# mapillary/OpenSfM

Hardware: NVIDIA H100
Metric: BA observations/sec (higher is better)
Workload: dtype f64

## Files before the change

### opensfm_b200/csrc/ba.cu

```cuda
#include <algorithm>
#include <dlfcn.h>

#include <chrono>
#include <cstring>
#include <mutex>
#include <cmath>
#include <cstdlib>
#include <string>
#include <vector>

#include "ba_models.cuh"
#include "common.cuh"

struct OsfmNcclId { char internal[128]; };

namespace osfm {

struct BAView {
  int K, NI, NR, S, P;
  long long N;
  int nc, npf;
  int wc, nres;
  int loss;
  double loss_a;
// ... 802 lines not shown
  osfm_allreduce_fn allreduce = nullptr;
  void* allreduce_user = nullptr;
  void* nccl_comm = nullptr;
  int nccl_rank = -1, nccl_world = 0;
  bool reproj_valid = false;
  osfm_ba_summary summary{};
  bool has_run = false;
  unsigned fallbacks = 0;
  int cap_iter = 0;
  bool cap_valid = false;
  osfm_ba_capture cap_info{};
  std::vector<double> cap_sbuf, cap_y, cap_scale, cap_diag, cap_grad;
  std::vector<double> cap_cam, cap_inst, cap_rc, cap_pts, cap_ext;
  std::vector<double> cap_side_r, cap_side_J;
  std::vector<int4> cap_upper;
  std::vector<int> cap_blk_off, cap_blk_sz, cap_pt_poff, cap_global_of;
  int cap_nc_pad = 0;
  bool cov_on = false, cov_ran = false, cov_valid = false;
  int cov_status = OSFM_COV_OK;
  double cov_pass_ms = 0.0, cov_chol_ms = 0.0;
  std::vector<double> cov_out;
  DevBuf<double> d_cov;
  DevBuf<int> d_cov_perm, d_cov_inst, d_cov_flags;

  DevBuf<int> d_cam_type, d_cam_off, d_cam_np, d_cam_poff, d_inst_poff, d_rc_poff, d_pt_poff;
  DevBuf<int> d_shot_inst, d_shot_cam, d_shot_rc, d_shot_use_rc, d_obs_shot, d_obs_point;
  DevBuf<double> d_obs_x, d_obs_y, d_obs_isig;
  DevBuf<long long> d_obs_orig, d_pt_start;
  DevBuf<double> d_cam[2], d_inst[2], d_rc[2], d_pts[2];
  DevBuf<double> d_r, d_Jc, d_Jp, d_Sbuf, d_Vinv, d_gp, d_slots;
  DevBuf<double> d_scale, d_colnorm2, d_grad, d_diag, d_y, d_bs_t;
  DevBuf<double> d_px, d_pr, d_pz, d_pp, d_pAp, d_Minv, d_reproj, d_full_pts;
  DevBuf<double> d_Wdef;
  DevBuf<int> d_blk_off, d_blk_sz, d_cam_blk, d_inst_blk, d_rc_blk;
  DevBuf<unsigned long long> d_tkeys, d_skeys, d_skeys2, d_rkeys, d_rkeys2;
  DevBuf<int> d_tvals, d_area, d_offs, d_row_ptr, d_row_col, d_row_off, d_diag_off, d_prior_diag_off;
  DevBuf<int> d_pr_blk, d_pr_local, d_g_obs_shot, d_g_obs_point;
  DevBuf<long long> d_g_pt_start;
  DevBuf<int4> d_upper;
  DevBuf<unsigned> d_count;
  DevBuf<char> d_cub;
  DevBuf<PcgState> d_pcg;
  DevBuf<int> d_seg_start;
  DevBuf<int> d_raw_shot, d_raw_point, d_ptc_full;
  DevBuf<double> d_raw_xy, d_raw_sigma, d_pts_in;
  DevBuf<unsigned long long> d_okeys, d_okeys2, d_pkey, d_pkey2;
  DevBuf<int> d_ovals, d_ovals2, d_pval, d_order, d_inv_order, d_global_of, d_free_flag, d_free_scan, d_head, d_run_head, d_nsel;
  DevBuf<long long> d_kk;
  DevBuf<char> d_seg_flags;
  DevBuf<OrderCounts> d_oc;
  PinnedBuf<OrderCounts> h_oc;
  DevBuf<double> d_rowsJ, d_rowsW, d_rowsY, d_Vig;
  DevBuf<int> d_row_M, d_qoff, d_blk_row, d_cbase, d_colidx, d_row_of, d_grp_b1, d_grp_b2;
  DevBuf<long long> d_rowbase;
  DevBuf<double> d_Spcg, d_Ap;
  PinnedBuf<PcgState> h_pcg;
  DevBuf<int> d_pcg_rowlo;
  DevBuf<int> d_pcg_grplo;
  DevBuf<char> d_grp_shared;
  DevBuf<unsigned long long> d_prof;
  DevBuf<long long> d_tab_off, d_tab_sizes;
  DevBuf<int> d_sp_nch, d_sp_chunk0;
  DevBuf<SchurChunk> d_sp_chunks;
  DevBuf<int> d_sp_ftab;
  DevBuf<int> d_tab;
  DevBuf<double> d_ptsum;
// ... 421 lines not shown
  upload(d_pr_cam_scale, rs.pr_cam_scale, stream); upload(d_pr_pos_inst, rs.pr_pos_inst, stream);
  upload(d_pr_pos_axis, rs.pr_pos_axis, stream); upload(d_pr_pos_col, rs.pr_pos_col, stream);
  upload(d_pr_pos_kind, rs.pr_pos_kind, stream);
  std::vector<double> ev = ext_values, el = ext_lower;
  if (ev.empty()) { ev.assign(1, 0.0); el.assign(1, 0.0); }
  upload(d_ext[0], ev, stream); upload(d_ext[1], ev, stream); upload(d_ext_lower, el, stream);
  upload(d_ext_off, rs.ext_off, stream); upload(d_ext_np, ext_size, stream); upload(d_ext_poff, rs.ext_poff, stream);
  upload(d_ext_blk, rs.ext_blk, stream);
  upload(d_side_terms, side_terms, stream); upload(d_side_consts, side_consts, stream);
  upload(d_side_jofs, rs.side_jofs, stream); upload(d_side_rofs, rs.side_rofs, stream);
  d_side_J.reserve((size_t)rs.side_jofs[NT] + 1); d_side_r.reserve((size_t)rs.side_rofs[NT] + 1);
  std::vector<double> ppd, ppx;
  if (rs.have_pp) {
    ppd.assign(3 * (size_t)Pfull, 0.0); ppx.assign(3 * (size_t)Pfull, 0.0);
    for (size_t q = 0; q < pp_point.size(); ++q) {
      const size_t g = (size_t)pp_point[q];
      for (int j = 0; j < (pp_alt[q] ? 3 : 2); ++j) {
        ppd[3 * g + j] = 1.0 / std::max(pp_sigma[3 * q + j], DBL_EPSILON);
        ppx[3 * g + j] = pp_prior[3 * q + j];
      }
    }
    upload(d_pp_d, ppd, stream); upload(d_pp_x0, ppx, stream);
  }
  OSFM_CUDA(cudaStreamSynchronize(stream));
  upload(d_pr_pos_prior, rs.pr_pos_prior, stream); upload(d_pr_pos_scale, rs.pr_pos_scale, stream);
  const size_t Nz = (size_t)std::max<long long>(rs.N, 1);
  d_r.reserve(nres * Nz); d_Jc.reserve((size_t)nres * wc * Nz); d_Jp.reserve((size_t)nres * 3 * Nz);
  d_Vinv.reserve(6 * (size_t)std::max(npf, 1)); d_gp.reserve(3 * (size_t)std::max(npf, 1));
  d_Vig.reserve(3 * (size_t)std::max(npf, 1)); d_bs_t.reserve(3 * (size_t)std::max(npf, 1));
  const size_t nz = rs.nz;
  d_scale.reserve(nz); d_colnorm2.reserve(nz); d_grad.reserve(nz); d_diag.reserve(nz); d_diag_r.reserve(nz); d_y.reserve(nz);
  d_px.reserve(std::max(nc, 1)); d_pr.reserve(std::max(nc, 1)); d_pz.reserve(std::max(nc, 1));
  d_pp.reserve(std::max(nc, 1)); d_pAp.reserve(std::max(nc, 1));
  d_pcg.reserve(1);
  d_Minv.reserve((size_t)std::max(rs.ngroups, 1) * MAXB * MAXB);
  d_Ap.reserve(std::max(nc, 1));
  d_sc.reserve(1);

  BAView& v = rs.v;
  v.K = rs.K; v.NI = rs.NI; v.NR = rs.NR; v.S = rs.S; v.P = P; v.N = rs.N; v.nc = nc; v.npf = npf; v.wc = wc; v.nres = nres;
  v.loss = loss; v.loss_a = loss_a;
  v.cam_type = d_cam_type.p; v.cam_off = d_cam_off.p; v.cam_np = d_cam_np.p; v.cam_poff = d_cam_poff.p;
  v.inst_poff = d_inst_poff.p; v.rc_poff = d_rc_poff.p; v.pt_poff = d_pt_poff.p;
  v.shot_inst = d_shot_inst.p; v.shot_cam = d_shot_cam.p; v.shot_rc = d_shot_rc.p; v.shot_use_rc = d_shot_use_rc.p;
  v.obs_shot = d_obs_shot.p; v.obs_point = d_obs_point.p; v.obs_x = d_obs_x.p; v.obs_y = d_obs_y.p;
  v.obs_isig = d_obs_isig.p; v.obs_orig = d_obs_orig.p; v.pt_start = d_pt_start.p;
  v.r = d_r.p; v.Jc = d_Jc.p; v.Jp = d_Jp.p;
  PriorView& pv = rs.pv;
  pv.n_cam_rows = rs.add_priors ? (int)rs.pr_cam_param.size() : 0;
  pv.n_pos_rows = rs.add_priors ? (int)rs.pr_pos_inst.size() : 0;
  pv.cam_row_param = d_pr_cam_param.p; pv.cam_row_col = d_pr_cam_col.p; pv.cam_row_log = d_pr_cam_log.p;
  pv.cam_row_prior = d_pr_cam_prior.p; pv.cam_row_scale = d_pr_cam_scale.p;
  pv.pos_row_kind = d_pr_pos_kind.p;
  pv.pos_row_inst = d_pr_pos_inst.p; pv.pos_row_axis = d_pr_pos_axis.p; pv.pos_row_col = d_pr_pos_col.p;
  pv.pos_row_prior = d_pr_pos_prior.p; pv.pos_row_scale = d_pr_pos_scale.p;
  SideView& sv = rs.sv;
  sv.n = NT; sv.terms = d_side_terms.p; sv.consts = d_side_consts.p; sv.jofs = d_side_jofs.p; sv.rofs = d_side_rofs.p;
  sv.J = d_side_J.p; sv.r = d_side_r.p;
  sv.ext_off = d_ext_off.p; sv.ext_np = d_ext_np.p; sv.ext_poff = d_ext_poff.p; sv.ext_blk = d_ext_blk.p;
  rs.ppv = PointPriorView{rs.have_pp ? d_pp_d.p : nullptr, d_pp_x0.p, d_global_of.p};
  rs.bm = BlkMaps{d_cam_blk.p, d_inst_blk.p, d_rc_blk.p};
}

void BA::discover_structure() {
  const int nblk = rs.nblk, nc = rs.nc, NT = rs.NT;
  if (nblk > 0) {
// ... 455 lines not shown
    if (timed) lm_phase(LM_PH_SCHUR, -1);
  }
  if (nc > 0) {
    if (world > 1) allreduce_dev(d_Sbuf.p, (long long)rs.nc_pad + rs.s_upper_total);
    PriorView pall = rs.pv;
    pall.n_cam_rows = (int)rs.pr_cam_param.size();
    pall.n_pos_rows = (int)rs.pr_pos_inst.size();
    const int nall = pall.n_cam_rows + pall.n_pos_rows;
    if (nall > 0) {
      ba_prior_system<<<grid_for(nall, 128), 128, 0, stream>>>(pall, params_of(0), d_scale.p, d_prior_diag_off.p,
                                                              d_S_p, d_rhs_p);
      OSFM_LAUNCH_CHECK();
    }
    if (rs.NT > 0) {
      side_system<<<rs.NT, SIDE_THREADS, 0, stream>>>(rs.sv, rs.v, rs.bm, params_of(0), rs.bsr, d_scale.p, d_S_p, d_rhs_p);
      OSFM_LAUNCH_CHECK();
    }
    ba_finish_system<<<grid_for((long long)rs.n_upper * 32, 256), 256, 0, stream>>>(d_upper.p, rs.n_upper, rs.bsr, d_S_p,
                                                                                  diag, inv_radius);
    OSFM_LAUNCH_CHECK();
  }
}

void BA::solve_reduced() {
  const int nc = rs.nc;
  lm_phase(-1, LM_PH_PCG);
  pcg_convert<<<grid_for((long long)rs.n_blocks_all * 32, 256), 256, 0, stream>>>(
      rs.d_S_p, d_row_col.p, d_row_off.p, d_qoff.p, d_blk_row.p, rs.n_blocks_all, rs.bsr, d_row_M.p, d_rowbase.p, d_Spcg.p);
  OSFM_LAUNCH_CHECK();
  pcg_factor_groups<<<grid_for((long long)rs.ngroups * 32, 32 * PFG_WARPS), 32 * PFG_WARPS, 0, stream>>>(rs.d_S_p, rs.bsr, d_diag_off.p, d_grp_b1.p, d_grp_b2.p,
                                                                rs.ngroups, d_Minv.p);
  OSFM_LAUNCH_CHECK();
  OSFM_CUDA(cudaMemsetAsync(d_pcg.p, 0, sizeof(PcgState), stream));
  const int max_pcg = std::min(2 * nc + 100, 5000);
  const int classic_path = rs.pcg_resident ? OSFM_PCG_CLASSIC_RESIDENT : OSFM_PCG_CLASSIC_STREAMED;
  auto classic = [&]() {
    launch_cooperative(rs.pcg_resident ? pcg_persistent<true> : pcg_persistent<false>, rs.pcg_grid, PCG_THREADS, rs.pcg_smem,
                       stream, d_Spcg.p, rs.lay, rs.bsr, d_Minv.p, rs.d_rhs_p, d_px.p, d_pr.p, d_pz.p, d_pp.p, d_pAp.p, d_Ap.p,
                       d_pcg.p, nc, max_pcg, 1e-16, rs.pcg_res);
    OSFM_LAUNCH_CHECK();
    if (tracing()) {
      OSFM_CUDA(cudaMemcpyAsync(h_pcg.p, d_pcg.p, PCG_STATE_HEADER, cudaMemcpyDeviceToHost, stream));
      OSFM_CUDA(cudaStreamSynchronize(stream));
      const PcgState& h = *h_pcg.p;
      const int its = std::max(h.iterations, 1);
      fprintf(stderr, "[osfm_ba] pcg %d its, CTA0 clocks/it: stage %lld matvec %lld reduce1 %lld phaseB %lld reduce2 %lld (resident %d)\n",
              h.iterations, h.prof[0] / its, h.prof[1] / its, h.prof[2] / its, h.prof[3] / its, h.prof[4] / its, (int)rs.pcg_resident);
    }
  };
  if (rs.pcg_pipe_ok) {
    launch_cooperative(pcg_pipelined, rs.pcg_grid, PCG_THREADS, rs.pcg_pipe_smem, stream, d_Spcg.p, rs.lay, rs.bsr, d_Minv.p,
                       rs.d_rhs_p, d_px.p, d_pz.p, d_pp.p, d_pcg.p, nc, max_pcg, 1e-16, rs.pcg_pipe);
    OSFM_LAUNCH_CHECK();
    if (tracing()) {
      OSFM_CUDA(cudaMemcpyAsync(h_pcg.p, d_pcg.p, PCG_STATE_HEADER, cudaMemcpyDeviceToHost, stream));
      OSFM_CUDA(cudaStreamSynchronize(stream));
      const PcgState& h = *h_pcg.p;
      const int its = std::max(h.iterations, 1);
      fprintf(stderr, "[osfm_ba] pipelined pcg %d its converged %d, CTA0 clocks/it: stage %lld matvec %lld reduce %lld update %lld"
              " | wide barrier (all calls / its): own sums %lld release %lld collect %lld column sums %lld\n",
              h.iterations, h.converged, h.prof[0] / its, h.prof[1] / its, h.prof[2] / its, h.prof[3] / its, h.prof[4] / its,
              h.prof[5] / its, h.prof[6] / its, h.prof[7] / its);
    }
    ba_lm_pcg_check<<<1, 1, 0, stream>>>(d_lm.p, d_pcg.p, classic_path, rs.h_pcg, rs.cap_graph != nullptr);
    OSFM_LAUNCH_CHECK();
    rs.k_pcg = lm_if(rs.h_pcg, LM_PCG_CLASSIC, [&]() {
      OSFM_CUDA(cudaMemsetAsync(d_pcg.p, 0, sizeof(PcgState), stream));
      classic();
    });
  } else {
    classic();
  }
  OSFM_CUDA(cudaMemcpyAsync(d_y.p, d_px.p, sizeof(double) * nc, cudaMemcpyDeviceToDevice, stream));
  lm_phase(LM_PH_PCG, -1);
}

void BA::back_substitute() {
  const int P = rs.P, npf = rs.npf;
  if (P == 0 || npf == 0) return;
  lm_phase(-1, LM_PH_BACK);
  OSFM_CUDA(cudaMemsetAsync(d_bs_t.p, 0, sizeof(double) * 3 * (size_t)npf, stream));
  if (rs.N > 0) {
    ba_backsub_rows<<<grid_for(rs.N, 256), 256, 0, stream>>>(rs.v, d_scale.p, d_y.p, d_bs_t.p);
    OSFM_LAUNCH_CHECK();
  }
  if (rs.have_pp) {
    ba_point_prior<3><<<grid_for(P, 128), 128, 0, stream>>>(rs.ppv, rs.v, params_of(0), nullptr, nullptr, d_bs_t.p, d_sc.p);
    OSFM_LAUNCH_CHECK();
  }
  ba_backsub_points<<<grid_for(npf, 256), 256, 0, stream>>>(rs.v, d_scale.p, d_Vinv.p, d_bs_t.p, d_y.p);
  OSFM_LAUNCH_CHECK();
  lm_phase(LM_PH_BACK, -1);
}

void BA::capture_linear_system(int it, double radius) {
// ... 772 lines not shown
```

### opensfm_b200/csrc/ba_reduced.cuh

```cuda
#pragma once
#include <cub/cub.cuh>

#include "ba_pcg_plan.h"

namespace osfm {

constexpr unsigned long long BSR_EMPTY = ~0ull;

struct BsrView {
  const unsigned long long* tkeys;
  const int* tvals;
  unsigned tmask;
  int nblk;
  const int* blk_off;
  const int* blk_sz;
};

__device__ __forceinline__ unsigned bsr_hash(unsigned long long k) {
  k ^= k >> 33; k *= 0xff51afd7ed558ccdULL; k ^= k >> 33; k *= 0xc4ceb9fe1a85ec53ULL; k ^= k >> 33;
  return (unsigned)k;
}
__device__ __forceinline__ int bsr_lookup(const BsrView& h, int bi, int bj) {
  const unsigned long long key = (unsigned long long)bi * (unsigned)h.nblk + (unsigned)bj;
  unsigned slot = bsr_hash(key) & h.tmask;
// ... 1116 lines not shown
      double s = L[i * MAXB + j];
      for (int k = 0; k < j; ++k) s -= L[i * MAXB + k] * L[j * MAXB + k];
      L[i * MAXB + j] = s / L[j * MAXB + j];
    }
    __syncwarp();
  }
  if (lane >= n) return;
  const int c = lane;
  double* out = Minv + (size_t)g * MAXB * MAXB;
  double y[MAXB];
  for (int i = 0; i < n; ++i) {
    double s = (i == c) ? 1.0 : 0.0;
    for (int k = 0; k < i; ++k) s -= L[i * MAXB + k] * y[k];
    y[i] = s / L[i * MAXB + i];
  }
  for (int i = n - 1; i >= 0; --i) {
    double s = y[i];
    for (int k = i + 1; k < n; ++k) s -= L[k * MAXB + i] * y[k];
    y[i] = s / L[i * MAXB + i];
  }
  for (int i = 0; i < n; ++i) out[i * MAXB + c] = y[i];
}

constexpr int PCG_MAX_CTAS = 256;
constexpr int PCG_FLAG_STRIDE = 32;
struct PcgState {
  int iterations;
  int converged;
  double rr_final;
  int deflated;
  long long prof[8];
  alignas(16) double slot[2][PCG_MAX_CTAS][4];
  double slotx[2][PCG_MAX_CTAS][12];
  unsigned flags[PCG_MAX_CTAS * PCG_FLAG_STRIDE];
};
constexpr size_t PCG_STATE_HEADER = offsetof(PcgState, slot);

struct PcgResident {
  const int* row_lo;
  int off_S, off_cols, off_rows;
  int max_rows;
};

__device__ __forceinline__ double ldcg_d(const double* p) { return __ldcg(p); }

template <int NV>
__device__ __forceinline__ void grid_reduce(PcgState* st, unsigned nblocks, unsigned& gen, double a, double b, double c,
                                            double& A, double& B, double& C, double (*red)[3]) {
  static_assert(NV == 2 || NV == 3, "two or three sums");
  ++gen;
  const int lane = threadIdx.x & 31, warp = threadIdx.x >> 5, nwarps = blockDim.x >> 5;
#pragma unroll
  for (int o = 16; o; o >>= 1) {
    a += __shfl_xor_sync(0xffffffffu, a, o);
    b += __shfl_xor_sync(0xffffffffu, b, o);
    if (NV == 3) c += __shfl_xor_sync(0xffffffffu, c, o);
  }
  if (lane == 0) { red[warp][0] = a; red[warp][1] = b; if (NV == 3) red[warp][2] = c; }
  __syncthreads();
  if (threadIdx.x == 0) {
    double sa = 0.0, sb = 0.0, sc = 0.0;
    for (int w = 0; w < nwarps; ++w) { sa += red[w][0]; sb += red[w][1]; if (NV == 3) sc += red[w][2]; }
    double* sl = st->slot[gen & 1][blockIdx.x];
    __stcg(reinterpret_cast<double2*>(sl), make_double2(sa, sb));
    if (NV == 3) __stcg(sl + 2, sc);
    asm volatile("st.release.gpu.global.u32 [%0], %1;" ::"l"(&st->flags[blockIdx.x * PCG_FLAG_STRIDE]), "r"(gen) : "memory");
// ... 212 lines not shown
                                  const double* __restrict__ scale, int nc, double* __restrict__ W) {
  const int i = blockIdx.x * blockDim.x + threadIdx.x;
  if (i >= NI) return;
  const int c0 = inst_poff[i];
  if (c0 < 0) return;
  const double r[3] = {inst[6 * (size_t)i], inst[6 * (size_t)i + 1], inst[6 * (size_t)i + 2]};
  const double t[3] = {inst[6 * (size_t)i + 3], inst[6 * (size_t)i + 4], inst[6 * (size_t)i + 5]};
  const double th2 = r[0] * r[0] + r[1] * r[1] + r[2] * r[2];
  double g = 1.0 / 12.0;
  if (th2 > 1e-8) {
    const double th = sqrt(th2);
    g = 1.0 / th2 - (1.0 + cos(th)) / (2.0 * th * sin(th));
  }
  const double K[9] = {0.0, -r[2], r[1], r[2], 0.0, -r[0], -r[1], r[0], 0.0};
  double J[9];
  for (int a = 0; a < 3; ++a)
    for (int b = 0; b < 3; ++b) {
      double k2 = 0.0;
      for (int c = 0; c < 3; ++c) k2 += K[a * 3 + c] * K[c * 3 + b];
      J[a * 3 + b] = (a == b ? 1.0 : 0.0) - 0.5 * K[a * 3 + b] + g * k2;
    }
  double inv_s[6];
  for (int j = 0; j < 6; ++j) inv_s[j] = 1.0 / scale[c0 + j];
  for (int a = 0; a < 3; ++a) {
    W[(size_t)a * nc + c0 + 3 + a] = inv_s[3 + a];
    for (int b = 0; b < 3; ++b) W[(size_t)(3 + a) * nc + c0 + b] = J[b * 3 + a] * inv_s[b];
    const int a1 = (a + 1) % 3, a2 = (a + 2) % 3;
    W[(size_t)(3 + a) * nc + c0 + 3 + a1] = -t[a2] * inv_s[3 + a1];
    W[(size_t)(3 + a) * nc + c0 + 3 + a2] = t[a1] * inv_s[3 + a2];
    W[(size_t)6 * nc + c0 + 3 + a] = t[a] * inv_s[3 + a];
  }
}

__device__ __noinline__ void grid_reduce_wide(PcgState* st, unsigned nblocks, unsigned* gen_io, double* vals ,
                                              double* gather , const double* inrow ,
                                              int nactive) {
  const unsigned gen = ++(*gen_io);
  const int lane = threadIdx.x & 31, warp = threadIdx.x >> 5;
  const bool probe = blockIdx.x == 0 && threadIdx.x == 0;
  long long tq = probe ? clock64() : 0;
  __syncthreads();
  if (warp < PCG_NW) {
    double sa = 0.0;
    for (int r = lane; r < nactive; r += 32) sa += inrow[r * PCG_NW + warp];
#pragma unroll
    for (int o = 16; o; o >>= 1) sa += __shfl_xor_sync(0xffffffffu, sa, o);
    if (lane == 0) __stcg(&st->slotx[gen & 1][blockIdx.x][warp], sa);
  }
  __syncthreads();
  if (probe) { const long long now = clock64(); st->prof[4] += now - tq; tq = now; }
  if (threadIdx.x == 0)
    asm volatile("st.release.gpu.global.u32 [%0], %1;" ::"l"(&st->flags[blockIdx.x * PCG_FLAG_STRIDE]), "r"(gen) : "memory");
  if (probe) { const long long now = clock64(); st->prof[5] += now - tq; tq = now; }
  if (threadIdx.x < nblocks) {
    const long long t0 = clock64();
    unsigned cur;
    do {
      asm volatile("ld.acquire.gpu.global.u32 %0, [%1];" : "=r"(cur) : "l"(&st->flags[threadIdx.x * PCG_FLAG_STRIDE]) : "memory");
      if (clock64() - t0 > 8000000000LL) __trap();
    } while ((int)(cur - gen) < 0);
    const double2* sl = reinterpret_cast<const double2*>(st->slotx[gen & 1][threadIdx.x]);
    double2 v[PCG_NW / 2];
#pragma unroll
    for (int i = 0; i < PCG_NW / 2; ++i) v[i] = __ldcg(sl + i);
    double2* dst = reinterpret_cast<double2*>(gather + threadIdx.x * PCG_NW);
#pragma unroll
    for (int i = 0; i < PCG_NW / 2; ++i) dst[i] = v[i];
  }
  __syncthreads();
  if (probe) { const long long now = clock64(); st->prof[6] += now - tq; tq = now; }
  if (warp < PCG_NW) {
    double sa = 0.0;
    for (unsigned c = lane; c < nblocks; c += 32) sa += gather[c * PCG_NW + warp];
#pragma unroll
    for (int o = 16; o; o >>= 1) sa += __shfl_xor_sync(0xffffffffu, sa, o);
    if (lane == 0) vals[warp] = sa;
  }
  __syncthreads();
  if (probe) st->prof[7] += clock64() - tq;
}
static_assert(PCG_THREADS / 32 >= PCG_NW, "a warp per value of the wide barrier");

__global__ void __launch_bounds__(PCG_THREADS, 1)
    pcg_pipelined(const double* __restrict__ Spcg, PcgLayout L, BsrView h, const double* __restrict__ Minv,
                  const double* __restrict__ rhs, double* __restrict__ x_out, double* mbuf0, double* mbuf1, PcgState* st,
                  int nc, int max_iter, double tol2_rel, PcgPipe R) {
  extern __shared__ __align__(16) unsigned char pcg_smem[];
  __shared__ double red[PCG_THREADS / 32][3];
  __shared__ int s_nrows, s_ncols;
  const int nwarps = blockDim.x >> 5, warp = threadIdx.x >> 5, lane = threadIdx.x & 31, tid = threadIdx.x;
  double* mp_s = reinterpret_cast<double*>(pcg_smem);
  double* S_s = reinterpret_cast<double*>(pcg_smem + R.off_S);
  double* Minv_s = reinterpret_cast<double*>(pcg_smem + R.off_Minv);
  double* w_s = reinterpret_cast<double*>(pcg_smem + R.off_vec);
  double* n_s = w_s + R.max_rows;
  double* g_s = n_s + R.max_rows;
  unsigned short* cols_s = reinterpret_cast<unsigned short*>(pcg_smem + R.off_cols);
  int* row_soff = reinterpret_cast<int*>(pcg_smem + R.off_rows);
  int* row_coff = row_soff + R.max_rows;
  int* row_len = row_coff + R.max_rows;
  int* row_gidx = row_len + R.max_rows;
  int* grp_row0 = row_gidx + R.max_rows;
  int* grp_moff = grp_row0 + R.max_groups + 1;
  int* unit_soff = grp_moff + R.max_groups + 1;
  int* unit_coff = unit_soff + R.max_rows;
  int* unit_len = unit_coff + R.max_rows;
  int* unit_lr0 = unit_len + R.max_rows;
  int* unit_nr = unit_lr0 + R.max_rows;
  __shared__ double part_s[PCG_THREADS / 8][3];
  __shared__ int s_nunits;
  __shared__ double redw[PCG_THREADS / 32][PCG_NW];
  __shared__ double Einv_s[PCG_ND * PCG_ND], c0_s[PCG_ND], tc_s[PCG_ND];
  __shared__ int s_defl;
  double* Wd_s = reinterpret_cast<double*>(pcg_smem + R.off_defl);
  double* AW_s = Wd_s + PCG_ND * R.max_rows;
  double* gather_s = AW_s + PCG_ND * R.max_rows;
  double* inrow_s = gather_s + PCG_NW * gridDim.x;
  double* wide_s = &redw[0][0];
  const int MR = R.max_rows;
  double* mbuf[2] = {mbuf0, mbuf1};
  unsigned bar_gen = 0;

  const int g_lo = R.grp_lo[blockIdx.x], g_hi = R.grp_lo[blockIdx.x + 1], ng = g_hi - g_lo;
  if (tid == 0) {
    int lr = 0, s_off = 0, c_off = 0, m_off = 0;
    for (int g = g_lo; g < g_hi; ++g) {
      grp_row0[g - g_lo] = lr;
      grp_moff[g - g_lo] = m_off;
      const int lr0 = lr;
      for (int k = 0; k < 2; ++k) {
        const int b = k ? L.grp_b2[g] : L.grp_b1[g];
        if (b < 0) continue;
        const int n = h.blk_sz[b], M = L.row_M[b];
        if (k && R.grp_shared[g]) c_off -= M;
        for (int r = 0; r < n; ++r, ++lr) {
          row_soff[lr] = s_off + r * M;
          row_coff[lr] = c_off;
          row_len[lr] = M;
          row_gidx[lr] = h.blk_off[b] + r;
        }
        s_off += n * M;
        c_off += M;
      }
      m_off += (lr - lr0) * (lr - lr0);
    }
    grp_row0[ng] = lr;
    grp_moff[ng] = m_off;
    s_nrows = lr;
    s_ncols = c_off;
    int nu = 0;
    for (int r0 = 0; r0 < lr;) {
      int nr = 1;
      while (nr < 3 && r0 + nr < lr && row_coff[r0 + nr] == row_coff[r0] && row_soff[r0 + nr] == row_soff[r0] + nr * row_len[r0]) ++nr;
      unit_soff[nu] = row_soff[r0]; unit_coff[nu] = row_coff[r0]; unit_len[nu] = row_len[r0]; unit_lr0[nu] = r0; unit_nr[nu] = nr;
      ++nu;
      r0 += nr;
    }
    s_nunits = nu;
  }
  __syncthreads();
  const int nrows = s_nrows, ncols = s_ncols;
  for (int lr = warp; lr < nrows; lr += nwarps) {
    const int i = row_gidx[lr], b = L.row_of[i], M = row_len[lr];
    const double* src = Spcg + L.rowbase[b] + (long long)(i - h.blk_off[b]) * M;
    for (int q = lane; q < M; q += 32) S_s[row_soff[lr] + q] = __ldcs(src + q);
    if (i == h.blk_off[b] && (lr == 0 || row_coff[lr] != row_coff[lr - 1])) {
      const int* csrc = L.colidx + L.cbase[b];
      for (int q = lane; q < M; q += 32) cols_s[row_coff[lr] + q] = (unsigned short)csrc[q];
    }
  }
  for (int gl = warp; gl < ng; gl += nwarps) {
    const int n = grp_row0[gl + 1] - grp_row0[gl];
    const double* src = Minv + (size_t)(g_lo + gl) * MAXB * MAXB;
    for (int t = lane; t < n * n; t += 32) Minv_s[grp_moff[gl] + t] = src[(t / n) * MAXB + t % n];
  }

  auto group_solve = [&](double* publish) {
    for (int gl = warp; gl < ng; gl += nwarps) {
      const int r0 = grp_row0[gl], n = grp_row0[gl + 1] - r0;
      const double* M = Minv_s + grp_moff[gl];
      double sv = 0.0;
      if (lane < n)
        for (int j = 0; j < n; ++j) sv += M[lane * n + j] * w_s[r0 + j];
      if (lane < n) {
        g_s[r0 + lane] = sv;
        publish[row_gidx[r0 + lane]] = sv;
      }
    }
  };
  auto matvec = [&]() {
    const int nunits = s_nunits;
    const int gidx = tid >> 3, l = tid & 7, ngroups8 = blockDim.x >> 3;
    const int gpu = max(1, ngroups8 / nunits);
    for (int ub = 0; ub < nunits; ub += ngroups8) {
      const int upass = min(nunits - ub, ngroups8 / gpu);
      const int ul = gidx / gpu, sub = gidx - ul * gpu;
      const int u = ub + ul;
      double a0 = 0.0, a1 = 0.0, a2 = 0.0;
      const bool on = ul < upass;
      if (on) {
        const int M = unit_len[u], nr = unit_nr[u];
        const double* v0 = S_s + unit_soff[u];
        const double* v1 = v0 + (nr > 1 ? M : 0);
        const double* v2 = v0 + (nr > 2 ? 2 * M : 0);
        const double* mp = mp_s + unit_coff[u];
        const int step = gpu * 8;
        int q = sub * 8 + l;
        for (; q + step < M; q += 2 * step) {
          const double m0 = mp[q], m1 = mp[q + step];
          a0 += v0[q] * m0; a1 += v1[q] * m0; a2 += v2[q] * m0;
          a0 += v0[q + step] * m1; a1 += v1[q + step] * m1; a2 += v2[q + step] * m1;
        }
        if (q < M) { const double m0 = mp[q]; a0 += v0[q] * m0; a1 += v1[q] * m0; a2 += v2[q] * m0; }
      }
#pragma unroll
      for (int o = 4; o; o >>= 1) {
        a0 += __shfl_xor_sync(0xffffffffu, a0, o);
        a1 += __shfl_xor_sync(0xffffffffu, a1, o);
        a2 += __shfl_xor_sync(0xffffffffu, a2, o);
      }
      if (l == 0) { part_s[gidx][0] = a0; part_s[gidx][1] = a1; part_s[gidx][2] = a2; }
      __syncthreads();
      if (tid < upass * 3) {
        const int uu = tid / 3, r = tid - uu * 3;
        const int u2 = ub + uu;
        if (r < unit_nr[u2]) {
          double sv = 0.0;
          for (int g2 = 0; g2 < gpu; ++g2) sv += part_s[uu * gpu + g2][r];
          n_s[unit_lr0[u2] + r] = sv;
        }
      }
      __syncthreads();
    }
  };
  auto stage = [&](const double* src) {
    const int bd = blockDim.x;
    for (int e = tid; e < ncols; e += 8 * bd) {
      double a[8];
#pragma unroll
      for (int k = 0; k < 8; ++k) a[k] = (e + k * bd < ncols) ? ldcg_d(src + cols_s[e + k * bd]) : 0.0;
#pragma unroll
      for (int k = 0; k < 8; ++k)
        if (e + k * bd < ncols) mp_s[e + k * bd] = a[k];
    }
  };

  const bool mine = tid < nrows;
  const int gi = mine ? row_gidx[tid] : 0;
  const double bi = mine ? rhs[gi] : 0.0;
  bool defl = R.Wdef != nullptr;
  double bb;
  if (defl) {
    __syncthreads();
#pragma unroll 1
    for (int j = 0; j < PCG_ND; ++j) {
      if (mine) Wd_s[j * MR + tid] = R.Wdef[(size_t)j * nc + gi];
      stage(R.Wdef + (size_t)j * nc);
      __syncthreads();
      matvec();
      __syncthreads();
      if (mine) AW_s[j * MR + tid] = n_s[tid];
      __syncthreads();
    }
    double E[PCG_ND * PCG_ND], wb[PCG_ND];
    bb = 0.0;
    int e_idx = 0;
    double collected[40];
    for (int pass = 0; pass < 4; ++pass) {
#pragma unroll
      for (int q = 0; q < PCG_NW; ++q) {
        const int idx = pass * PCG_NW + q;
        double val = 0.0;
        if (mine) {
          if (idx < 28) {
            int a = 0, rem = idx;
            while (rem >= PCG_ND - a) { rem -= PCG_ND - a; ++a; }
            const int b2 = a + rem;
            val = Wd_s[a * MR + tid] * AW_s[b2 * MR + tid];
          } else if (idx < 35) {
            val = Wd_s[(idx - 28) * MR + tid] * bi;
          } else if (idx == 35) {
            val = bi * bi;
          }
        }
        if (mine) inrow_s[tid * PCG_NW + q] = val;
      }
      grid_reduce_wide(st, gridDim.x, &bar_gen, wide_s, gather_s, inrow_s, nrows);
#pragma unroll
      for (int q = 0; q < PCG_NW; ++q) collected[pass * PCG_NW + q] = wide_s[q];
      __syncthreads();
    }
    (void)e_idx;
    if (tid == 0) {
      int idx = 0;
      for (int a = 0; a < PCG_ND; ++a)
        for (int b2 = a; b2 < PCG_ND; ++b2) { E[a * PCG_ND + b2] = collected[idx]; E[b2 * PCG_ND + a] = collected[idx]; ++idx; }
      for (int a = 0; a < PCG_ND; ++a) wb[a] = collected[28 + a];
      double Lc[PCG_ND * PCG_ND];
      bool ok = true;
      double dmax = 0.0;
      for (int a = 0; a < PCG_ND; ++a) dmax = fmax(dmax, E[a * PCG_ND + a]);
      for (int j = 0; j < PCG_ND && ok; ++j) {
        double dd = E[j * PCG_ND + j];
        for (int k2 = 0; k2 < j; ++k2) dd -= Lc[j * PCG_ND + k2] * Lc[j * PCG_ND + k2];
        if (!(dd > 1e-12 * dmax) || !(dmax > 0.0)) { ok = false; break; }
        dd = sqrt(dd);
        Lc[j * PCG_ND + j] = dd;
        for (int i2 = j + 1; i2 < PCG_ND; ++i2) {
          double sv2 = E[i2 * PCG_ND + j];
          for (int k2 = 0; k2 < j; ++k2) sv2 -= Lc[i2 * PCG_ND + k2] * Lc[j * PCG_ND + k2];
          Lc[i2 * PCG_ND + j] = sv2 / dd;
        }
      }
      if (ok) {
        for (int cidx = 0; cidx < PCG_ND; ++cidx) {
          double y[PCG_ND];
          for (int i2 = 0; i2 < PCG_ND; ++i2) {
            double sv2 = (i2 == cidx) ? 1.0 : 0.0;
            for (int k2 = 0; k2 < i2; ++k2) sv2 -= Lc[i2 * PCG_ND + k2] * y[k2];
            y[i2] = sv2 / Lc[i2 * PCG_ND + i2];
          }
          for (int i2 = PCG_ND - 1; i2 >= 0; --i2) {
            double sv2 = y[i2];
            for (int k2 = i2 + 1; k2 < PCG_ND; ++k2) sv2 -= Lc[k2 * PCG_ND + i2] * y[k2];
            y[i2] = sv2 / Lc[i2 * PCG_ND + i2];
          }
          for (int i2 = 0; i2 < PCG_ND; ++i2) Einv_s[i2 * PCG_ND + cidx] = y[i2];
        }
        for (int a = 0; a < PCG_ND; ++a) {
          double sv2 = 0.0;
          for (int b2 = 0; b2 < PCG_ND; ++b2) sv2 += Einv_s[a * PCG_ND + b2] * wb[b2];
          c0_s[a] = sv2;
        }
      }
      s_defl = ok ? 1 : 0;
    }
    __syncthreads();
    bb = collected[35];
    defl = s_defl != 0;
  }
  auto coarse = [&]() {
    if (tid < PCG_ND) {
      double sv2 = 0.0;
#pragma unroll
      for (int b2 = 0; b2 < PCG_ND; ++b2) sv2 += Einv_s[tid * PCG_ND + b2] * wide_s[3 + b2];
      tc_s[tid] = sv2;
    }
    __syncthreads();
  };
  auto aw_dot = [&](const double* c) -> double {
    double sv2 = 0.0;
#pragma unroll
    for (int j = 0; j < PCG_ND; ++j) sv2 += AW_s[j * MR + tid] * c[j];
    return sv2;
  };

  double xr = 0.0, rr_ = bi, u = 0.0, w = 0.0, z = 0.0, q = 0.0, sv_ = 0.0, p = 0.0;
  if (defl && mine) rr_ = bi - aw_dot(c0_s);
  if (mine) w_s[tid] = rr_;
  __syncthreads();
  group_solve(mbuf[0]);
  if (defl) {
    __syncthreads();
    if (mine) {
      double* ir = inrow_s + tid * PCG_NW;
      ir[0] = 0.0; ir[1] = 0.0; ir[2] = 0.0;
#pragma unroll
      for (int j = 0; j < PCG_ND; ++j) ir[3 + j] = AW_s[j * MR + tid] * g_s[tid];
    }
    grid_reduce_wide(st, gridDim.x, &bar_gen, wide_s, gather_s, inrow_s, nrows);
    coarse();
  } else {
    double d0, d1, d2;
    grid_reduce<3>(st, gridDim.x, bar_gen, 0.0, 0.0, mine ? rr_ * rr_ : 0.0, d0, d1, d2, red);
    bb = d2;
  }
  const double tol2 = tol2_rel * bb;
  double rr = bb;
  int it = 0, converged = 0;
  if (bb > 0.0) {
    if (mine) u = g_s[tid];
    stage(mbuf[0]);
    __syncthreads();
    matvec();
    __syncthreads();
    if (mine) { w = n_s[tid] - (defl ? aw_dot(tc_s) : 0.0); w_s[tid] = w; }
    __syncthreads();
    group_solve(mbuf[1]);
    double gamma_prev = 1.0, alpha_prev = 1.0, best = bb;
    int since_best = 0;
    for (;; ++it) {
      const long long tk0 = clock64();
      double gamma, delta;
      if (defl) {
        __syncthreads();
        if (mine) {
          double* ir = inrow_s + tid * PCG_NW;
          ir[0] = rr_ * u; ir[1] = w * u; ir[2] = rr_ * rr_;
#pragma unroll
          for (int j = 0; j < PCG_ND; ++j) ir[3 + j] = AW_s[j * MR + tid] * g_s[tid];
        }
        grid_reduce_wide(st, gridDim.x, &bar_gen, wide_s, gather_s, inrow_s, nrows);
        gamma = wide_s[0]; delta = wide_s[1]; rr = wide_s[2];
        coarse();
      } else
        grid_reduce<3>(st, gridDim.x, bar_gen, mine ? rr_ * u : 0.0, mine ? w * u : 0.0, mine ? rr_ * rr_ : 0.0, gamma, delta, rr,
                   red);
      const long long tk1 = clock64();
      if (!(rr == rr)) break;
      if (rr <= tol2) { converged = 1; break; }
      if (rr < best) { best = rr; since_best = 0; } else if (++since_best > 150) break;
      if (it >= max_iter) break;
      const double* mcur = mbuf[(it + 1) & 1];
      stage(mcur);
      __syncthreads();
      const long long tk2 = clock64();
      matvec();
      __syncthreads();
      const long long tk3 = clock64();
      const double beta = it > 0 ? gamma / gamma_prev : 0.0;
      const double alpha = it > 0 ? gamma / (delta - beta * gamma / alpha_prev) : gamma / delta;
      if (mine) {
        const double mo = g_s[tid], nn = n_s[tid] - (defl ? aw_dot(tc_s) : 0.0);
        z = nn + beta * z;
        q = mo + beta * q;
        sv_ = w + beta * sv_;
        p = u + beta * p;
        xr += alpha * p;
        rr_ -= alpha * sv_;
        u -= alpha * q;
        w -= alpha * z;
        w_s[tid] = w;
      }
      __syncthreads();
      group_solve(mbuf[it & 1]);
      gamma_prev = gamma;
      alpha_prev = alpha;
      if (blockIdx.x == 0 && tid == 0) {
        const long long tk4 = clock64();
        st->prof[0] += tk2 - tk1; st->prof[1] += tk3 - tk2; st->prof[2] += tk1 - tk0; st->prof[3] += tk4 - tk3;
      }
    }
  } else {
    converged = 1;
  }
  if (defl) {
    if (mine) {
      double* ir = inrow_s + tid * PCG_NW;
      ir[0] = 0.0; ir[1] = 0.0; ir[2] = 0.0;
#pragma unroll
      for (int j = 0; j < PCG_ND; ++j) ir[3 + j] = AW_s[j * MR + tid] * xr;
    }
    grid_reduce_wide(st, gridDim.x, &bar_gen, wide_s, gather_s, inrow_s, nrows);
    coarse();
    if (mine) {
      double add = 0.0;
#pragma unroll
      for (int j = 0; j < PCG_ND; ++j) add += Wd_s[j * MR + tid] * (c0_s[j] - tc_s[j]);
      xr += add;
    }
  }
  if (mine) x_out[gi] = xr;
  if (converged && bb > 0.0) {
    if (mine) mbuf[0][gi] = xr;
    double d0, d1, d2;
    grid_reduce<3>(st, gridDim.x, bar_gen, 0.0, 0.0, 0.0, d0, d1, d2, red);
    stage(mbuf[0]);
    __syncthreads();
    matvec();
    __syncthreads();
    const double tr = mine ? bi - n_s[tid] : 0.0;
    grid_reduce<3>(st, gridDim.x, bar_gen, 0.0, 0.0, tr * tr, d0, d1, d2, red);
    rr = d2;
    if (!(rr <= 4.0 * tol2)) converged = 0;
  }
  if (blockIdx.x == 0 && tid == 0) {
    st->iterations = it; st->rr_final = rr; st->converged = converged; st->deflated = defl ? 1 : 0;
  }
}

}
```

Measured before the change: 720.6 million.

## Replace pipelined PCG grid barriers with generation-tagged flag values and split post/collect

Replaces the grid-wide barrier reductions in the pipelined PCG loop with per-value flags that carry a generation tag. Each CTA posts its partial sums, stages the preconditioned vector and runs the matvec, and only afterwards collects the reduced dot products. The staged vector entries are also published as tagged words, so consumers spin on the data itself rather than on a separate barrier. This lets the reduction latency overlap with stage and matvec, at the cost of doubled storage for the tagged words, an extra memset per solve, spin-wait loops, and more intricate memory-ordering reasoning.

```diff
diff --git a/opensfm_b200/csrc/ba.cu b/opensfm_b200/csrc/ba.cu
--- a/opensfm_b200/csrc/ba.cu
+++ b/opensfm_b200/csrc/ba.cu
@@ -858,6 +858,7 @@
   DevBuf<double> d_scale, d_colnorm2, d_grad, d_diag, d_y, d_bs_t;
   DevBuf<double> d_px, d_pr, d_pz, d_pp, d_pAp, d_Minv, d_reproj, d_full_pts;
   DevBuf<double> d_Wdef;
+  DevBuf<unsigned long long> d_pm;
   DevBuf<int> d_blk_off, d_blk_sz, d_cam_blk, d_inst_blk, d_rc_blk;
   DevBuf<unsigned long long> d_tkeys, d_skeys, d_skeys2, d_rkeys, d_rkeys2;
   DevBuf<int> d_tvals, d_area, d_offs, d_row_ptr, d_row_col, d_row_off, d_diag_off, d_prior_diag_off;
@@ -1345,6 +1346,7 @@
   d_scale.reserve(nz); d_colnorm2.reserve(nz); d_grad.reserve(nz); d_diag.reserve(nz); d_diag_r.reserve(nz); d_y.reserve(nz);
   d_px.reserve(std::max(nc, 1)); d_pr.reserve(std::max(nc, 1)); d_pz.reserve(std::max(nc, 1));
   d_pp.reserve(std::max(nc, 1)); d_pAp.reserve(std::max(nc, 1));
+  d_pm.reserve(4 * (size_t)std::max(nc, 1));
   d_pcg.reserve(1);
   d_Minv.reserve((size_t)std::max(rs.ngroups, 1) * MAXB * MAXB);
   d_Ap.reserve(std::max(nc, 1));
@@ -1866,6 +1868,7 @@
                                                                 rs.ngroups, d_Minv.p);
   OSFM_LAUNCH_CHECK();
   OSFM_CUDA(cudaMemsetAsync(d_pcg.p, 0, sizeof(PcgState), stream));
+  if (rs.pcg_pipe_ok) OSFM_CUDA(cudaMemsetAsync(d_pm.p, 0, sizeof(unsigned long long) * 4 * (size_t)nc, stream));
   const int max_pcg = std::min(2 * nc + 100, 5000);
   const int classic_path = rs.pcg_resident ? OSFM_PCG_CLASSIC_RESIDENT : OSFM_PCG_CLASSIC_STREAMED;
   auto classic = [&]() {
@@ -1884,17 +1887,16 @@
   };
   if (rs.pcg_pipe_ok) {
     launch_cooperative(pcg_pipelined, rs.pcg_grid, PCG_THREADS, rs.pcg_pipe_smem, stream, d_Spcg.p, rs.lay, rs.bsr, d_Minv.p,
-                       rs.d_rhs_p, d_px.p, d_pz.p, d_pp.p, d_pcg.p, nc, max_pcg, 1e-16, rs.pcg_pipe);
+                       rs.d_rhs_p, d_px.p, d_pm.p, d_pcg.p, nc, max_pcg, 1e-16, rs.pcg_pipe);
     OSFM_LAUNCH_CHECK();
     if (tracing()) {
       OSFM_CUDA(cudaMemcpyAsync(h_pcg.p, d_pcg.p, PCG_STATE_HEADER, cudaMemcpyDeviceToHost, stream));
       OSFM_CUDA(cudaStreamSynchronize(stream));
       const PcgState& h = *h_pcg.p;
       const int its = std::max(h.iterations, 1);
-      fprintf(stderr, "[osfm_ba] pipelined pcg %d its converged %d, CTA0 clocks/it: stage %lld matvec %lld reduce %lld update %lld"
-              " | wide barrier (all calls / its): own sums %lld release %lld collect %lld column sums %lld\n",
-              h.iterations, h.converged, h.prof[0] / its, h.prof[1] / its, h.prof[2] / its, h.prof[3] / its, h.prof[4] / its,
-              h.prof[5] / its, h.prof[6] / its, h.prof[7] / its);
+      fprintf(stderr, "[osfm_ba] pipelined pcg %d its converged %d, CTA0 clocks/it: post %lld stage %lld matvec %lld collect %lld"
+              " update %lld\n", h.iterations, h.converged, h.prof[0] / its, h.prof[1] / its, h.prof[2] / its, h.prof[3] / its,
+              h.prof[4] / its);
     }
     ba_lm_pcg_check<<<1, 1, 0, stream>>>(d_lm.p, d_pcg.p, classic_path, rs.h_pcg, rs.cap_graph != nullptr);
     OSFM_LAUNCH_CHECK();
diff --git a/opensfm_b200/csrc/ba_reduced.cuh b/opensfm_b200/csrc/ba_reduced.cuh
--- a/opensfm_b200/csrc/ba_reduced.cuh
+++ b/opensfm_b200/csrc/ba_reduced.cuh
@@ -1172,6 +1172,8 @@
   long long prof[8];
   alignas(16) double slot[2][PCG_MAX_CTAS][4];
   double slotx[2][PCG_MAX_CTAS][12];
+  alignas(16) unsigned long long slotf[2][PCG_NW][PCG_MAX_CTAS][2];
+  alignas(128) unsigned long long totf[2][PCG_NW][16];
   unsigned flags[PCG_MAX_CTAS * PCG_FLAG_STRIDE];
 };
 constexpr size_t PCG_STATE_HEADER = offsetof(PcgState, slot);
@@ -1450,13 +1452,23 @@
   }
 }
 
+__device__ __forceinline__ void wide_column_sums(unsigned nblocks, double* vals , const double* gather) {
+  const int lane = threadIdx.x & 31, warp = threadIdx.x >> 5;
+  if (warp < PCG_NW) {
+    double sa = 0.0;
+    for (unsigned c = lane; c < nblocks; c += 32) sa += gather[c * PCG_NW + warp];
+#pragma unroll
+    for (int o = 16; o; o >>= 1) sa += __shfl_xor_sync(0xffffffffu, sa, o);
+    if (lane == 0) vals[warp] = sa;
+  }
+  __syncthreads();
+}
+
 __device__ __noinline__ void grid_reduce_wide(PcgState* st, unsigned nblocks, unsigned* gen_io, double* vals ,
                                               double* gather , const double* inrow ,
                                               int nactive) {
   const unsigned gen = ++(*gen_io);
   const int lane = threadIdx.x & 31, warp = threadIdx.x >> 5;
-  const bool probe = blockIdx.x == 0 && threadIdx.x == 0;
-  long long tq = probe ? clock64() : 0;
   __syncthreads();
   if (warp < PCG_NW) {
     double sa = 0.0;
@@ -1466,10 +1478,8 @@
     if (lane == 0) __stcg(&st->slotx[gen & 1][blockIdx.x][warp], sa);
   }
   __syncthreads();
-  if (probe) { const long long now = clock64(); st->prof[4] += now - tq; tq = now; }
   if (threadIdx.x == 0)
     asm volatile("st.release.gpu.global.u32 [%0], %1;" ::"l"(&st->flags[blockIdx.x * PCG_FLAG_STRIDE]), "r"(gen) : "memory");
-  if (probe) { const long long now = clock64(); st->prof[5] += now - tq; tq = now; }
   if (threadIdx.x < nblocks) {
     const long long t0 = clock64();
     unsigned cur;
@@ -1486,22 +1496,131 @@
     for (int i = 0; i < PCG_NW / 2; ++i) dst[i] = v[i];
   }
   __syncthreads();
-  if (probe) { const long long now = clock64(); st->prof[6] += now - tq; tq = now; }
+  wide_column_sums(nblocks, vals, gather);
+}
+static_assert(PCG_THREADS / 32 >= PCG_NW, "a warp per value of the wide barrier");
+
+__device__ __forceinline__ void flag_put(unsigned long long* p, double v, unsigned gen) {
+  const unsigned long long b = (unsigned long long)__double_as_longlong(v), g = (unsigned long long)gen << 32;
+  asm volatile("st.relaxed.gpu.global.v2.b64 [%0], {%1, %2};" ::"l"(p), "l"((b & 0xffffffffull) | g), "l"((b >> 32) | g)
+               : "memory");
+}
+__device__ __forceinline__ ulonglong2 flag_ld(const unsigned long long* p) {
+  ulonglong2 w;
+  asm volatile("ld.relaxed.gpu.global.v2.b64 {%0, %1}, [%2];" : "=l"(w.x), "=l"(w.y) : "l"(p));
+  return w;
+}
+__device__ __forceinline__ bool flag_ok(ulonglong2 w, unsigned gen) {
+  return (unsigned)(w.x >> 32) == gen && (unsigned)(w.y >> 32) == gen;
+}
+__device__ __forceinline__ double flag_val(ulonglong2 w) {
+  return __longlong_as_double((long long)((w.x & 0xffffffffull) | (w.y << 32)));
+}
+template <int N, class Addr>
+__device__ __forceinline__ void flag_wait_all(ulonglong2 (&w)[N], Addr addr, unsigned gen) {
+  bool ok = true;
+#pragma unroll
+  for (int i = 0; i < N; ++i) ok = ok && flag_ok(w[i], gen);
+  if (ok) return;
+  const long long t0 = clock64();
+  do {
+#pragma unroll
+    for (int i = 0; i < N; ++i)
+      if (!flag_ok(w[i], gen)) w[i] = flag_ld(addr(i));
+    if (clock64() - t0 > 8000000000LL) __trap();
+    ok = true;
+#pragma unroll
+    for (int i = 0; i < N; ++i) ok = ok && flag_ok(w[i], gen);
+  } while (!ok);
+}
+
+__device__ __noinline__ void pcg_post_wide(PcgState* st, unsigned gen, const double* inrow ,
+                                           int nactive) {
+  const int lane = threadIdx.x & 31, warp = threadIdx.x >> 5;
+  __syncthreads();
   if (warp < PCG_NW) {
     double sa = 0.0;
-    for (unsigned c = lane; c < nblocks; c += 32) sa += gather[c * PCG_NW + warp];
+    for (int r = lane; r < nactive; r += 32) sa += inrow[r * PCG_NW + warp];
 #pragma unroll
     for (int o = 16; o; o >>= 1) sa += __shfl_xor_sync(0xffffffffu, sa, o);
-    if (lane == 0) vals[warp] = sa;
+    if (lane == 0) flag_put(st->slotf[gen & 1][warp][blockIdx.x], sa, gen);
+  }
+}
+__device__ __noinline__ void pcg_collect_wide(PcgState* st, unsigned nblocks, unsigned gen, double* vals ) {
+  const int lane = threadIdx.x & 31, warp = threadIdx.x >> 5;
+  const unsigned i = warp * nblocks + blockIdx.x;
+  if (i < PCG_NW) {
+    const unsigned long long(*sl)[2] = st->slotf[gen & 1][i];
+    const unsigned long long none = (unsigned long long)gen << 32;
+    constexpr int K = PCG_MAX_CTAS / 32;
+    ulonglong2 v[K];
+#pragma unroll
+    for (int k = 0; k < K; ++k) v[k] = lane + 32 * k < (int)nblocks ? flag_ld(sl[lane + 32 * k]) : make_ulonglong2(none, none);
+    flag_wait_all(v, [&](int k) { return sl[lane + 32 * k]; }, gen);
+    double sa = 0.0;
+#pragma unroll
+    for (int k = 0; k < K; ++k)
+      if (lane + 32 * k < (int)nblocks) sa += flag_val(v[k]);
+#pragma unroll
+    for (int o = 16; o; o >>= 1) sa += __shfl_xor_sync(0xffffffffu, sa, o);
+    if (lane == 0) flag_put(st->totf[gen & 1][i], sa, gen);
+  }
+  if (threadIdx.x < PCG_NW) {
+    ulonglong2 t[1] = {flag_ld(st->totf[gen & 1][threadIdx.x])};
+    flag_wait_all(t, [&](int) { return st->totf[gen & 1][threadIdx.x]; }, gen);
+    vals[threadIdx.x] = flag_val(t[0]);
   }
   __syncthreads();
-  if (probe) st->prof[7] += clock64() - tq;
-}
-static_assert(PCG_THREADS / 32 >= PCG_NW, "a warp per value of the wide barrier");
+}
+static_assert(PCG_MAX_CTAS % 32 == 0 && PCG_NW <= PCG_THREADS / 32, "pcg_collect_wide: whole warps of slots, a warp per value");
+
+__device__ __forceinline__ void pcg_post3(PcgState* st, unsigned gen, double a, double b, double c, double (*red)[3]) {
+  const int lane = threadIdx.x & 31, warp = threadIdx.x >> 5, nwarps = blockDim.x >> 5;
+#pragma unroll
+  for (int o = 16; o; o >>= 1) {
+    a += __shfl_xor_sync(0xffffffffu, a, o);
+    b += __shfl_xor_sync(0xffffffffu, b, o);
+    c += __shfl_xor_sync(0xffffffffu, c, o);
+  }
+  if (lane == 0) { red[warp][0] = a; red[warp][1] = b; red[warp][2] = c; }
+  __syncthreads();
+  if (threadIdx.x == 0) {
+    double sa = 0.0, sb = 0.0, sc = 0.0;
+    for (int w = 0; w < nwarps; ++w) { sa += red[w][0]; sb += red[w][1]; sc += red[w][2]; }
+    flag_put(st->slotf[gen & 1][0][blockIdx.x], sa, gen);
+    flag_put(st->slotf[gen & 1][1][blockIdx.x], sb, gen);
+    flag_put(st->slotf[gen & 1][2][blockIdx.x], sc, gen);
+  }
+  __syncthreads();
+}
+__device__ __forceinline__ void pcg_collect3(PcgState* st, unsigned nblocks, unsigned gen, double& A, double& B, double& C,
+                                             double (*red)[3]) {
+  const int lane = threadIdx.x & 31, warp = threadIdx.x >> 5;
+  double va = 0.0, vb = 0.0, vc = 0.0;
+  if (threadIdx.x < nblocks) {
+    const auto sl = st->slotf[gen & 1];
+    ulonglong2 v[3] = {flag_ld(sl[0][threadIdx.x]), flag_ld(sl[1][threadIdx.x]), flag_ld(sl[2][threadIdx.x])};
+    flag_wait_all(v, [&](int i) { return sl[i][threadIdx.x]; }, gen);
+    va = flag_val(v[0]); vb = flag_val(v[1]); vc = flag_val(v[2]);
+  }
+#pragma unroll
+  for (int o = 16; o; o >>= 1) {
+    va += __shfl_xor_sync(0xffffffffu, va, o);
+    vb += __shfl_xor_sync(0xffffffffu, vb, o);
+    vc += __shfl_xor_sync(0xffffffffu, vc, o);
+  }
+  if (lane == 0) { red[warp][0] = va; red[warp][1] = vb; red[warp][2] = vc; }
+  __syncthreads();
+  double sa = 0.0, sb = 0.0, sc = 0.0;
+  const int wmax = (int)((nblocks + 31) >> 5);
+  for (int w = 0; w < wmax; ++w) { sa += red[w][0]; sb += red[w][1]; sc += red[w][2]; }
+  A = sa; B = sb; C = sc;
+  __syncthreads();
+}
 
 __global__ void __launch_bounds__(PCG_THREADS, 1)
     pcg_pipelined(const double* __restrict__ Spcg, PcgLayout L, BsrView h, const double* __restrict__ Minv,
-                  const double* __restrict__ rhs, double* __restrict__ x_out, double* mbuf0, double* mbuf1, PcgState* st,
+                  const double* __restrict__ rhs, double* x_out, unsigned long long* mflag, PcgState* st,
                   int nc, int max_iter, double tol2_rel, PcgPipe R) {
   extern __shared__ __align__(16) unsigned char pcg_smem[];
   __shared__ double red[PCG_THREADS / 32][3];
@@ -1536,7 +1655,6 @@
   double* inrow_s = gather_s + PCG_NW * gridDim.x;
   double* wide_s = &redw[0][0];
   const int MR = R.max_rows;
-  double* mbuf[2] = {mbuf0, mbuf1};
   unsigned bar_gen = 0;
 
   const int g_lo = R.grp_lo[blockIdx.x], g_hi = R.grp_lo[blockIdx.x + 1], ng = g_hi - g_lo;
@@ -1593,7 +1711,8 @@
     for (int t = lane; t < n * n; t += 32) Minv_s[grp_moff[gl] + t] = src[(t / n) * MAXB + t % n];
   }
 
-  auto group_solve = [&](double* publish) {
+  auto group_solve = [&](unsigned gen) {
+    unsigned long long* publish = mflag + (size_t)(gen & 1) * 2 * nc;
     for (int gl = warp; gl < ng; gl += nwarps) {
       const int r0 = grp_row0[gl], n = grp_row0[gl + 1] - r0;
       const double* M = Minv_s + grp_moff[gl];
@@ -1602,7 +1721,7 @@
         for (int j = 0; j < n; ++j) sv += M[lane * n + j] * w_s[r0 + j];
       if (lane < n) {
         g_s[r0 + lane] = sv;
-        publish[row_gidx[r0 + lane]] = sv;
+        flag_put(publish + 2 * row_gidx[r0 + lane], sv, gen);
       }
     }
   };
@@ -1662,6 +1781,20 @@
         if (e + k * bd < ncols) mp_s[e + k * bd] = a[k];
     }
   };
+  auto stage_m = [&](unsigned gen) {
+    const unsigned long long* src = mflag + (size_t)(gen & 1) * 2 * nc;
+    const int bd = blockDim.x;
+    for (int e = tid; e < ncols; e += 8 * bd) {
+      const unsigned long long none = (unsigned long long)gen << 32;
+      ulonglong2 a[8];
+#pragma unroll
+      for (int k = 0; k < 8; ++k) a[k] = e + k * bd < ncols ? flag_ld(src + 2 * cols_s[e + k * bd]) : make_ulonglong2(none, none);
+      flag_wait_all(a, [&](int k) { return src + 2 * cols_s[e + k * bd]; }, gen);
+#pragma unroll
+      for (int k = 0; k < 8; ++k)
+        if (e + k * bd < ncols) mp_s[e + k * bd] = flag_val(a[k]);
+    }
+  };
 
   const bool mine = tid < nrows;
   const int gi = mine ? row_gidx[tid] : 0;
@@ -1681,9 +1814,7 @@
       __syncthreads();
     }
     double E[PCG_ND * PCG_ND], wb[PCG_ND];
-    bb = 0.0;
-    int e_idx = 0;
-    double collected[40];
+    double* collected = Einv_s;
     for (int pass = 0; pass < 4; ++pass) {
 #pragma unroll
       for (int q = 0; q < PCG_NW; ++q) {
@@ -1704,11 +1835,11 @@
         if (mine) inrow_s[tid * PCG_NW + q] = val;
       }
       grid_reduce_wide(st, gridDim.x, &bar_gen, wide_s, gather_s, inrow_s, nrows);
-#pragma unroll
-      for (int q = 0; q < PCG_NW; ++q) collected[pass * PCG_NW + q] = wide_s[q];
+      if (tid < PCG_NW && pass * PCG_NW + tid < 36) collected[pass * PCG_NW + tid] = wide_s[tid];
       __syncthreads();
     }
-    (void)e_idx;
+    bb = collected[35];
+    __syncthreads();
     if (tid == 0) {
       int idx = 0;
       for (int a = 0; a < PCG_ND; ++a)
@@ -1754,7 +1885,6 @@
       s_defl = ok ? 1 : 0;
     }
     __syncthreads();
-    bb = collected[35];
     defl = s_defl != 0;
   }
   auto coarse = [&]() {
@@ -1777,7 +1907,7 @@
   if (defl && mine) rr_ = bi - aw_dot(c0_s);
   if (mine) w_s[tid] = rr_;
   __syncthreads();
-  group_solve(mbuf[0]);
+  group_solve(1);
   if (defl) {
     __syncthreads();
     if (mine) {
@@ -1798,18 +1928,18 @@
   int it = 0, converged = 0;
   if (bb > 0.0) {
     if (mine) u = g_s[tid];
-    stage(mbuf[0]);
+    stage_m(1);
     __syncthreads();
     matvec();
     __syncthreads();
     if (mine) { w = n_s[tid] - (defl ? aw_dot(tc_s) : 0.0); w_s[tid] = w; }
     __syncthreads();
-    group_solve(mbuf[1]);
+    group_solve(2);
     double gamma_prev = 1.0, alpha_prev = 1.0, best = bb;
     int since_best = 0;
     for (;; ++it) {
+      const unsigned gen = (unsigned)it + 2u;
       const long long tk0 = clock64();
-      double gamma, delta;
       if (defl) {
         __syncthreads();
         if (mine) {
@@ -1818,24 +1948,28 @@
 #pragma unroll
           for (int j = 0; j < PCG_ND; ++j) ir[3 + j] = AW_s[j * MR + tid] * g_s[tid];
         }
-        grid_reduce_wide(st, gridDim.x, &bar_gen, wide_s, gather_s, inrow_s, nrows);
-        gamma = wide_s[0]; delta = wide_s[1]; rr = wide_s[2];
-        coarse();
+        pcg_post_wide(st, gen, inrow_s, nrows);
       } else
-        grid_reduce<3>(st, gridDim.x, bar_gen, mine ? rr_ * u : 0.0, mine ? w * u : 0.0, mine ? rr_ * rr_ : 0.0, gamma, delta, rr,
-                   red);
+        pcg_post3(st, gen, mine ? rr_ * u : 0.0, mine ? w * u : 0.0, mine ? rr_ * rr_ : 0.0, red);
       const long long tk1 = clock64();
-      if (!(rr == rr)) break;
-      if (rr <= tol2) { converged = 1; break; }
-      if (rr < best) { best = rr; since_best = 0; } else if (++since_best > 150) break;
-      if (it >= max_iter) break;
-      const double* mcur = mbuf[(it + 1) & 1];
-      stage(mcur);
+      stage_m(gen);
       __syncthreads();
       const long long tk2 = clock64();
       matvec();
       __syncthreads();
       const long long tk3 = clock64();
+      double gamma, delta;
+      if (defl) {
+        pcg_collect_wide(st, gridDim.x, gen, wide_s);
+        gamma = wide_s[0]; delta = wide_s[1]; rr = wide_s[2];
+        coarse();
+      } else
+        pcg_collect3(st, gridDim.x, gen, gamma, delta, rr, red);
+      const long long tk4 = clock64();
+      if (!(rr == rr)) break;
+      if (rr <= tol2) { converged = 1; break; }
+      if (rr < best) { best = rr; since_best = 0; } else if (++since_best > 150) break;
+      if (it >= max_iter) break;
       const double beta = it > 0 ? gamma / gamma_prev : 0.0;
       const double alpha = it > 0 ? gamma / (delta - beta * gamma / alpha_prev) : gamma / delta;
       if (mine) {
@@ -1851,12 +1985,13 @@
         w_s[tid] = w;
       }
       __syncthreads();
-      group_solve(mbuf[it & 1]);
+      group_solve(gen + 1);
       gamma_prev = gamma;
       alpha_prev = alpha;
       if (blockIdx.x == 0 && tid == 0) {
-        const long long tk4 = clock64();
-        st->prof[0] += tk2 - tk1; st->prof[1] += tk3 - tk2; st->prof[2] += tk1 - tk0; st->prof[3] += tk4 - tk3;
+        const long long tk5 = clock64();
+        st->prof[0] += tk1 - tk0; st->prof[1] += tk2 - tk1; st->prof[2] += tk3 - tk2; st->prof[3] += tk4 - tk3;
+        st->prof[4] += tk5 - tk4;
       }
     }
   } else {
@@ -1880,10 +2015,9 @@
   }
   if (mine) x_out[gi] = xr;
   if (converged && bb > 0.0) {
-    if (mine) mbuf[0][gi] = xr;
     double d0, d1, d2;
     grid_reduce<3>(st, gridDim.x, bar_gen, 0.0, 0.0, 0.0, d0, d1, d2, red);
-    stage(mbuf[0]);
+    stage(x_out);
     __syncthreads();
     matvec();
     __syncthreads();
```

Result: faster. 750.3 million (median of 6 runs) (+4.1%).
